# Zehong-Ma/MagCache

Hardware: NVIDIA H100
Metric: denoising_steps_per_sec (higher is better)
Workload: dtype bf16

## Files before the change

### magcache_b200/csrc/gemm_wgmma.cu

```cuda
#include <cstdlib>

#include "common.cuh"
#include "ptx.cuh"
#include "tma_host.cuh"

namespace mc {

TmapCacheEntry* tmap_cache() {
  static TmapCacheEntry table[kTmapCacheSize] = {};
  return table;
}
std::mutex& tmap_cache_mutex() {
  static std::mutex m;
  return m;
}

constexpr int kCluster = 2;
constexpr int kBM = 128, kBK = 64, kStages = 4;
constexpr int kClusterBM = kCluster * kBM;
constexpr int kTileABytes = kBM * kBK * 2;
constexpr int kStagePad = 33;
constexpr int kEpiWarps = 8;
constexpr int kPatchRows = 16;
constexpr int kStagingBytes = kEpiWarps * kPatchRows * kStagePad * 4;
constexpr int kGemmThreads = 128 + 32 * kEpiWarps;
constexpr int kProducerRegs = 40, kConsumerRegs = 232;
template <int BN>
struct GemmTile {
  static constexpr int kTileBBytes = BN * kBK * 2;
  static constexpr int kHalfBBytes = kTileBBytes / kCluster;
  static constexpr int kStageBytes = kTileABytes + kTileBBytes;
  static constexpr int kOffStaging = kStages * kStageBytes;
  static constexpr int kOffBars = kOffStaging + kStagingBytes;
  static constexpr int kSmem = kOffBars + 128;
};

struct GemmParams {
  int M, N, K;
  const float* bias;
  void* out;
  int64_t ldo;
  const float* gate;
  int total_tiles;
};

template <int EPI, int ROWS>
__device__ __forceinline__ void epilogue_patch(const GemmParams& p, const float* stage, int row0, int col0, int lane) {
  const int rows = min(ROWS, p.M - row0);
  if (rows <= 0) return;
  const int col = col0 + lane;
  const bool col_ok = col < p.N;

  if (EPI == MC_EPI_BIAS_GATE_RESID) {
    const float b = (p.bias && col_ok) ? p.bias[col] : 0.f;
    const float g = (p.gate && col_ok) ? p.gate[col] : 1.f;
    float* xcol = static_cast<float*>(p.out) + static_cast<int64_t>(row0) * p.ldo + col;
#pragma unroll
    for (int h = 0; h < ROWS; h += 16) {
      float xv[16];
#pragma unroll
      for (int r = 0; r < 16; ++r) xv[r] = (col_ok && h + r < rows) ? xcol[static_cast<int64_t>(h + r) * p.ldo] : 0.f;
#pragma unroll
      for (int r = 0; r < 16; ++r) {
        const float y = round_bf16(stage[(h + r) * kStagePad + lane] + b);
        xv[r] = __fadd_rn(xv[r], __fmul_rn(y, g));
      }
#pragma unroll
      for (int r = 0; r < 16; ++r)
        if (col_ok && h + r < rows) xcol[static_cast<int64_t>(h + r) * p.ldo] = xv[r];
    }
    return;
  }

  if (EPI == MC_EPI_BIAS_F32) {
    const float b = (p.bias && col_ok) ? p.bias[col] : 0.f;
    float* ocol = static_cast<float*>(p.out) + static_cast<int64_t>(row0) * p.ldo + col;
#pragma unroll
    for (int r = 0; r < ROWS; ++r)
      if (col_ok && r < rows) ocol[static_cast<int64_t>(r) * p.ldo] = stage[r * kStagePad + lane] + b;
    return;
  }

  const int half = lane >> 4, cp = (lane & 15) * 2;
  const int c0 = col0 + cp;
  float b0 = 0.f, b1 = 0.f;
  if (EPI != MC_EPI_ROWBIAS_BF16 && p.bias) {
    if (c0 < p.N) b0 = p.bias[c0];
    if (c0 + 1 < p.N) b1 = p.bias[c0 + 1];
  }
  float g0 = 1.f, g1 = 1.f;
  if (EPI == MC_EPI_BIAS_GATE_RESID_BF16 && p.gate) {
    if (c0 < p.N) g0 = p.gate[c0];
    if (c0 + 1 < p.N) g1 = p.gate[c0 + 1];
  }
  __nv_bfloat16* obase = static_cast<__nv_bfloat16*>(p.out) + static_cast<int64_t>(row0 + half) * p.ldo + c0;
  const float* sbase = stage + half * kStagePad + cp;
  const float* rbias = (EPI == MC_EPI_ROWBIAS_BF16 && p.bias) ? p.bias + row0 + half : nullptr;

  if (rows == ROWS && col0 + 32 <= p.N && (p.ldo & 1) == 0) {
    uint32_t w[ROWS / 2];
#pragma unroll
    for (int i = 0; i < ROWS / 2; ++i) {
      float v0 = sbase[2 * i * kStagePad], v1 = sbase[2 * i * kStagePad + 1];
      if (EPI == MC_EPI_ROWBIAS_BF16) {
        const float rb = rbias ? rbias[2 * i] : 0.f;
        v0 += rb;
        v1 += rb;
      } else {
        v0 += b0;
        v1 += b1;
      }
      if (EPI == MC_EPI_BIAS_GELU_BF16) {
        v0 = gelu_tanh(round_bf16(v0));
        v1 = gelu_tanh(round_bf16(v1));
      }
      if (EPI == MC_EPI_BIAS_GELU_ERF_BF16) {
        v0 = gelu_erf(round_bf16(v0));
        v1 = gelu_erf(round_bf16(v1));
      }
      if (EPI == MC_EPI_BIAS_SILU_BF16) {
        v0 = silu_f(round_bf16(v0));
        v1 = silu_f(round_bf16(v1));
      }
      if (EPI == MC_EPI_BIAS_GATE_RESID_BF16) {
        const uint32_t old = *reinterpret_cast<const uint32_t*>(obase + static_cast<int64_t>(2 * i) * p.ldo);
        v0 = bf16_lo(old) + round_bf16(g0 * round_bf16(v0));
        v1 = bf16_hi(old) + round_bf16(g1 * round_bf16(v1));
      }
      w[i] = pack_bf16x2(v0, v1);
    }
#pragma unroll
    for (int i = 0; i < ROWS / 2; ++i) *reinterpret_cast<uint32_t*>(obase + static_cast<int64_t>(2 * i) * p.ldo) = w[i];
    return;
  }

  const bool pair_ok = (c0 + 1 < p.N) && ((p.ldo & 1) == 0);
  for (int i = 0; i < ROWS / 2; ++i) {
    const int r = 2 * i + half;
    if (r >= rows) continue;
    float v0 = sbase[2 * i * kStagePad], v1 = sbase[2 * i * kStagePad + 1];
    if (EPI == MC_EPI_ROWBIAS_BF16) {
      const float rb = rbias ? rbias[2 * i] : 0.f;
      v0 += rb;
      v1 += rb;
    } else {
      v0 += b0;
      v1 += b1;
    }
    if (EPI == MC_EPI_BIAS_GELU_BF16) {
      v0 = gelu_tanh(round_bf16(v0));
      v1 = gelu_tanh(round_bf16(v1));
    }
    if (EPI == MC_EPI_BIAS_GELU_ERF_BF16) {
      v0 = gelu_erf(round_bf16(v0));
      v1 = gelu_erf(round_bf16(v1));
    }
    if (EPI == MC_EPI_BIAS_SILU_BF16) {
      v0 = silu_f(round_bf16(v0));
      v1 = silu_f(round_bf16(v1));
    }
    __nv_bfloat16* o = obase + static_cast<int64_t>(2 * i) * p.ldo;
    if (EPI == MC_EPI_BIAS_GATE_RESID_BF16) {
      if (c0 < p.N) v0 = __bfloat162float(o[0]) + round_bf16(g0 * round_bf16(v0));
      if (c0 + 1 < p.N) v1 = __bfloat162float(o[1]) + round_bf16(g1 * round_bf16(v1));
    }
    if (pair_ok) {
      *reinterpret_cast<uint32_t*>(o) = pack_bf16x2(v0, v1);
    } else {
      if (c0 < p.N) o[0] = __float2bfloat16_rn(v0);
      if (c0 + 1 < p.N) o[1] = __float2bfloat16_rn(v1);
    }
  }
}

template <int EPI, int kBN>
__global__ void __cluster_dims__(kCluster, 1, 1) __launch_bounds__(kGemmThreads, 1)
    gemm_bf16_kernel(const __grid_constant__ CUtensorMap tmap_a, const __grid_constant__ CUtensorMap tmap_b, const GemmParams p) {
  using T = GemmTile<kBN>;
  constexpr int kStageBytes = T::kStageBytes, kOffStaging = T::kOffStaging, kOffBars = T::kOffBars;
  extern __shared__ __align__(1024) uint8_t smem[];
  float* staging = reinterpret_cast<float*>(smem + kOffStaging);
  uint64_t* full_bar = reinterpret_cast<uint64_t*>(smem + kOffBars);
  uint64_t* empty_bar = full_bar + kStages;

  const int warp = threadIdx.x >> 5, lane = threadIdx.x & 31;
  const int n_tiles = (p.N + kBN - 1) / kBN;
  const int num_kb = (p.K + kBK - 1) / kBK;
  const uint32_t rank = ptx::cluster_ctarank();
  const int cluster = static_cast<int>(ptx::cluster_id_x()), n_clusters = static_cast<int>(ptx::num_clusters_x());
  const int steps = (p.total_tiles - cluster + n_clusters - 1) / n_clusters;

  if (threadIdx.x == 0) {
    if ((ptx::smem_u32(smem) & 1023u) != 0) {
      MC_DIAG("gemm_bf16_kernel: dynamic smem base not 1024-aligned\n");
      __trap();
    }
    ptx::prefetch_tmap(&tmap_a);
    ptx::prefetch_tmap(&tmap_b);
    for (int s = 0; s < kStages; ++s) {
      ptx::mbar_init(&full_bar[s], 1);
      ptx::mbar_init(&empty_bar[s], kCluster * kEpiWarps);
    }
    ptx::fence_mbar_init();
  }
  ptx::cluster_arrive();
  ptx::cluster_wait();

  if (warp < 4) {
    ptx::setmaxnreg_dec<kProducerRegs>();
    if (warp == 0) {
      uint32_t it = 0;
      for (int i = 0; i < steps; ++i) {
        const int tile = cluster + i * n_clusters;
        const int m0 = (tile / n_tiles) * kClusterBM + static_cast<int>(rank) * kBM, n0 = (tile % n_tiles) * kBN;
        const int nb = n0 + static_cast<int>(rank) * (kBN / kCluster);
        for (int kb = 0; kb < num_kb; ++kb, ++it) {
          const int s = it % kStages;
          const uint32_t ph = (it / kStages) & 1;
          ptx::mbar_wait(&empty_bar[s], ph ^ 1);
          if (ptx::elect_one()) {
            uint8_t* sa = smem + s * kStageBytes;
            ptx::mbar_expect_tx(&full_bar[s], kStageBytes);
            ptx::tma_load_2d(sa, &tmap_a, &full_bar[s], kb * kBK, m0);
            ptx::tma_load_2d_multicast(sa + kTileABytes + rank * T::kHalfBBytes, &tmap_b, &full_bar[s], kb * kBK, nb,
                                       static_cast<uint16_t>((1u << kCluster) - 1));
          }
          __syncwarp();
        }
      }
    }
  } else {
    ptx::setmaxnreg_inc<kConsumerRegs>();
    const int wg = (warp >> 2) - 1;
    const int wq = warp & 3;
    float acc[kBN / 2];
    bool timed_out = false;
    for (int i = 0; i < steps; ++i) {
      const int tile = cluster + i * n_clusters;
      const int m0 = (tile / n_tiles) * kClusterBM + static_cast<int>(rank) * kBM, n0 = (tile % n_tiles) * kBN;
      uint32_t it = static_cast<uint32_t>(i) * num_kb;
      int prev_s = -1;
      for (int kb = 0; kb < num_kb; ++kb, ++it) {
        const int s = it % kStages;
        const uint32_t ph = (it / kStages) & 1;
        ptx::mbar_wait_or_flag(&full_bar[s], ph, timed_out);
        const uint32_t sa = ptx::smem_u32(smem + s * kStageBytes);
        const uint64_t da = ptx::gmma_desc_sw128_kmajor(sa + wg * (64 * 128));
        const uint64_t db = ptx::gmma_desc_sw128_kmajor(sa + kTileABytes);
        ptx::wgmma_fence();
#pragma unroll
        for (int k = 0; k < kBK / 16; ++k) {
          if constexpr (kBN == 256) {
            ptx::wgmma_m64n256k16_ss(acc, da + 2 * k, db + 2 * k, (kb | k) != 0 ? 1u : 0u);
          } else {
            ptx::wgmma_m64n128k16_ss(acc, da + 2 * k, db + 2 * k, (kb | k) != 0 ? 1u : 0u);
          }
        }
        ptx::wgmma_commit();
        ptx::wgmma_wait<1>();
        ptx::fence_regs(acc);
        if (prev_s >= 0 && lane == 0)
          for (uint32_t c = 0; c < kCluster; ++c) ptx::mbar_arrive_cluster(&empty_bar[prev_s], c);
        prev_s = s;
      }
      ptx::wgmma_wait<0>();
      ptx::fence_regs(acc);
      if (lane == 0)
        for (uint32_t c = 0; c < kCluster; ++c) ptx::mbar_arrive_cluster(&empty_bar[prev_s], c);

      float* patch = staging + (4 * wg + wq) * kPatchRows * kStagePad;
      const int row0 = m0 + wg * 64 + wq * kPatchRows;
      const int r_lo = lane >> 2;
#pragma unroll
      for (int c = 0; c < kBN / 32; ++c) {
        __syncwarp();
#pragma unroll
        for (int q = 0; q < 4; ++q) {
          const int i = 4 * c + q;
          const int col = 8 * q + 2 * (lane & 3);
          patch[r_lo * kStagePad + col] = acc[4 * i + 0];
          patch[r_lo * kStagePad + col + 1] = acc[4 * i + 1];
          patch[(r_lo + 8) * kStagePad + col] = acc[4 * i + 2];
          patch[(r_lo + 8) * kStagePad + col + 1] = acc[4 * i + 3];
        }
        __syncwarp();
        epilogue_patch<EPI, kPatchRows>(p, patch, row0, n0 + c * 32, lane);
      }
    }
    if (timed_out) __trap();
  }
  ptx::cluster_arrive();
  ptx::cluster_wait();
}

template <int EPI, int BN>
static int32_t max_active_clusters(int* out) {
  static int cached[kMaxDevices] = {};
  const int d = current_device();
  if (cached[d] > 0) {
    *out = cached[d];
    return MC_OK;
  }
  cudaLaunchConfig_t cfg = {};
  cfg.gridDim = dim3(kCluster * num_sms(), 1, 1);
  cfg.blockDim = dim3(kGemmThreads, 1, 1);
  cfg.dynamicSmemBytes = GemmTile<BN>::kSmem;
  int n = 0;
  const cudaError_t e = cudaOccupancyMaxActiveClusters(&n, gemm_bf16_kernel<EPI, BN>, &cfg);
  if (e != cudaSuccess) return cuda_fail(e, "cudaOccupancyMaxActiveClusters(gemm)");
  if (n < 1) {
    set_error("gemm_bf16_kernel: no cluster of %d CTAs with %d B of shared memory fits on this device", kCluster, GemmTile<BN>::kSmem);
    return MC_ERR_CUDA;
  }
  cached[d] = n;
  *out = n;
  return MC_OK;
}

template <int EPI, int BN>
static int32_t launch_gemm_bn(const CUtensorMap& ta, const CUtensorMap& tb, GemmParams p, cudaStream_t s) {
  static PerDeviceOnce once;
  int32_t rc = set_max_smem_once(gemm_bf16_kernel<EPI, BN>, GemmTile<BN>::kSmem, once, "cudaFuncSetAttribute(gemm smem)");
  if (rc) return rc;
  int clusters = 0;
  rc = max_active_clusters<EPI, BN>(&clusters);
  if (rc) return rc;
  const int m_tiles = (p.M + kClusterBM - 1) / kClusterBM, n_tiles = (p.N + BN - 1) / BN;
  const int total = m_tiles * n_tiles;
  p.total_tiles = total;
  const int grid = kCluster * (total < clusters ? total : clusters);
  gemm_bf16_kernel<EPI, BN><<<grid, kGemmThreads, GemmTile<BN>::kSmem, s>>>(ta, tb, p);
  MC_CHECK_LAUNCH("gemm_bf16_kernel launch");
  return MC_OK;
}

static int pick_bn(int M, int N) {
  const char* e = getenv("MC_GEMM_BN");
  if (e && *e) {
    const int v = atoi(e);
    if (v == 128 || v == 256) return v;
  }
  const int64_t sms = num_sms(), m_tiles = (M + 127) / 128;
  const int64_t t256 = m_tiles * ((N + 255) / 256), t128 = m_tiles * ((N + 127) / 128);
  const int64_t cost256 = ((t256 + sms - 1) / sms) * 100, cost128 = ((t128 + sms - 1) / sms) * 62;
  return cost128 * 100 <= cost256 * 92 ? 128 : 256;
}

}

extern "C" int32_t mc_gemm_bf16(const void* A, int64_t lda, const void* B, int64_t ldb, int32_t M, int32_t N, int32_t K,
                                const float* bias, int32_t epilogue, void* out, int64_t ldo, const float* gate, void* stream) {
  MC_CHECK_ARG(A && B && out, "mc_gemm_bf16: null pointer");
  MC_CHECK_ARG(M >= 1 && N >= 1 && K >= 8, "mc_gemm_bf16: M=%d N=%d K=%d", M, N, K);
  MC_CHECK_ARG(K % 8 == 0 && lda % 8 == 0 && ldb % 8 == 0 && lda >= K && ldb >= K, "mc_gemm_bf16: K/lda/ldb must be multiples of 8 (16-byte TMA pitch)");
  MC_CHECK_ARG(mc::aligned16(A) && mc::aligned16(B) && mc::aligned16(out), "mc_gemm_bf16: A/B/out must be 16-byte aligned");
  MC_CHECK_ARG(ldo >= N, "mc_gemm_bf16: ldo=%lld < N=%d", static_cast<long long>(ldo), N);
  CUtensorMap ta, tb;
  int32_t rc = mc::make_tmap_bf16_2d(&ta, A, static_cast<uint64_t>(M), static_cast<uint64_t>(K), static_cast<uint64_t>(lda), mc::kBM, mc::kBK);
  if (rc) return rc;
  const int bn = mc::pick_bn(M, N);
  rc = mc::make_tmap_bf16_2d(&tb, B, static_cast<uint64_t>(N), static_cast<uint64_t>(K), static_cast<uint64_t>(ldb), bn / mc::kCluster,
                             mc::kBK);
  if (rc) return rc;
  mc::GemmParams p{M, N, K, bias, out, ldo, gate, 0};
  cudaStream_t s = static_cast<cudaStream_t>(stream);
#define MC_GEMM_CASE(E) \
  case E: return bn == 128 ? mc::launch_gemm_bn<E, 128>(ta, tb, p, s) : mc::launch_gemm_bn<E, 256>(ta, tb, p, s)
  switch (epilogue) {
    MC_GEMM_CASE(MC_EPI_BIAS_BF16);
    MC_GEMM_CASE(MC_EPI_BIAS_GELU_BF16);
    MC_GEMM_CASE(MC_EPI_BIAS_GATE_RESID);
    MC_GEMM_CASE(MC_EPI_ROWBIAS_BF16);
    MC_GEMM_CASE(MC_EPI_BIAS_F32);
    MC_GEMM_CASE(MC_EPI_BIAS_GELU_ERF_BF16);
    MC_GEMM_CASE(MC_EPI_BIAS_GATE_RESID_BF16);
    MC_GEMM_CASE(MC_EPI_BIAS_SILU_BF16);
#undef MC_GEMM_CASE
    default:
      mc::set_error("mc_gemm_bf16: unknown epilogue %d", epilogue);
      return MC_ERR_INVALID;
  }
}
```

### magcache_b200/csrc/ptx.cuh

```cuda
#pragma once
#include <cstdint>
#include <cuda_runtime.h>

namespace ptx {

__device__ __forceinline__ uint32_t smem_u32(const void* p) {
  return static_cast<uint32_t>(__cvta_generic_to_shared(p));
}

__device__ __forceinline__ void mbar_init(uint64_t* bar, uint32_t count) {
  asm volatile("mbarrier.init.shared::cta.b64 [%0], %1;" ::"r"(smem_u32(bar)), "r"(count) : "memory");
}
__device__ __forceinline__ void fence_mbar_init() {
  asm volatile("fence.mbarrier_init.release.cluster;" ::: "memory");
}
__device__ __forceinline__ void mbar_expect_tx(uint64_t* bar, uint32_t bytes) {
  asm volatile("mbarrier.arrive.expect_tx.shared::cta.b64 _, [%0], %1;" ::"r"(smem_u32(bar)), "r"(bytes) : "memory");
}
__device__ __forceinline__ void mbar_arrive(uint64_t* bar) {
  asm volatile("mbarrier.arrive.shared::cta.b64 _, [%0];" ::"r"(smem_u32(bar)) : "memory");
}
__device__ __forceinline__ bool mbar_try_wait(uint64_t* bar, uint32_t parity) {
  uint32_t ok;
  asm volatile(
      "{\n"
      ".reg .pred p;\n"
      "mbarrier.try_wait.parity.shared::cta.b64 p, [%1], %2;\n"
      "selp.u32 %0, 1, 0, p;\n"
      "}\n"
      : "=r"(ok)
      : "r"(smem_u32(bar)), "r"(parity)
      : "memory");
  return ok != 0;
}
#ifndef MC_DEVICE_DIAG
#define MC_DEVICE_DIAG 0
#endif
#if MC_DEVICE_DIAG
#define MC_DIAG(...) printf(__VA_ARGS__)
#else
#define MC_DIAG(...) ((void)0)
#endif

#ifndef MC_MBAR_TIMEOUT_CYCLES
#define MC_MBAR_TIMEOUT_CYCLES (4000000000ll)
#endif
__device__ __forceinline__ void mbar_wait(uint64_t* bar, uint32_t parity) {
  if (mbar_try_wait(bar, parity)) return;
  const long long t0 = clock64();
  while (!mbar_try_wait(bar, parity)) {
    if (clock64() - t0 > MC_MBAR_TIMEOUT_CYCLES) {
      MC_DIAG("mbar_wait timeout: block (%d,%d,%d) thread %d bar smem+%u parity %u\n", blockIdx.x, blockIdx.y, blockIdx.z,
              threadIdx.x, smem_u32(bar), parity);
      __trap();
    }
  }
}
__device__ __forceinline__ void mbar_wait_or_flag(uint64_t* bar, uint32_t parity, bool& timed_out) {
  if (timed_out || mbar_try_wait(bar, parity)) return;
  const long long t0 = clock64();
  while (!mbar_try_wait(bar, parity)) {
    if (clock64() - t0 > MC_MBAR_TIMEOUT_CYCLES) {
      MC_DIAG("mbar_wait timeout: block (%d,%d,%d) thread %d bar smem+%u parity %u\n", blockIdx.x, blockIdx.y, blockIdx.z,
              threadIdx.x, smem_u32(bar), parity);
      timed_out = true;
      return;
    }
  }
}

__device__ __forceinline__ void named_bar_sync(uint32_t id, uint32_t count) {
  asm volatile("bar.sync %0, %1;" ::"r"(id), "r"(count) : "memory");
}
__device__ __forceinline__ void named_bar_arrive(uint32_t id, uint32_t count) {
  asm volatile("bar.arrive %0, %1;" ::"r"(id), "r"(count) : "memory");
}

__device__ __forceinline__ uint32_t cluster_ctarank() {
  uint32_t r;
  asm volatile("mov.u32 %0, %%cluster_ctarank;" : "=r"(r));
  return r;
}
__device__ __forceinline__ uint32_t cluster_id_x() {
  uint32_t r;
  asm volatile("mov.u32 %0, %%clusterid.x;" : "=r"(r));
  return r;
}
__device__ __forceinline__ uint32_t num_clusters_x() {
  uint32_t r;
  asm volatile("mov.u32 %0, %%nclusterid.x;" : "=r"(r));
  return r;
}
__device__ __forceinline__ void mbar_arrive_cluster(uint64_t* bar, uint32_t cta) {
  asm volatile(
      "{\n"
      ".reg .b32 ra;\n"
      "mapa.shared::cluster.u32 ra, %0, %1;\n"
      "mbarrier.arrive.shared::cluster.b64 _, [ra];\n"
      "}\n"
      ::"r"(smem_u32(bar)), "r"(cta)
      : "memory");
}
__device__ __forceinline__ void cluster_arrive() { asm volatile("barrier.cluster.arrive.release.aligned;" ::: "memory"); }
__device__ __forceinline__ void cluster_wait() { asm volatile("barrier.cluster.wait.acquire.aligned;" ::: "memory"); }

__device__ __forceinline__ bool elect_one() {
  uint32_t pred;
  asm volatile(
      "{\n"
      ".reg .pred P;\n"
      "elect.sync _|P, 0xffffffff;\n"
      "selp.u32 %0, 1, 0, P;\n"
      "}\n"
      : "=r"(pred));
  return pred != 0;
}

__device__ __forceinline__ void fence_proxy_async_smem() {
  asm volatile("fence.proxy.async.shared::cta;" ::: "memory");
}

__device__ __forceinline__ void prefetch_tmap(const void* tmap) {
  asm volatile("prefetch.tensormap [%0];" ::"l"(reinterpret_cast<uint64_t>(tmap)) : "memory");
}
__device__ __forceinline__ void tma_load_2d(void* smem_dst, const void* tmap, uint64_t* bar, int32_t c0, int32_t c1) {
  asm volatile(
      "cp.async.bulk.tensor.2d.shared::cluster.global.mbarrier::complete_tx::bytes [%0], [%1, {%3, %4}], [%2];"
      ::"r"(smem_u32(smem_dst)), "l"(reinterpret_cast<uint64_t>(tmap)), "r"(smem_u32(bar)), "r"(c0), "r"(c1)
      : "memory");
}

__device__ __forceinline__ void tma_load_2d_multicast(void* smem_dst, const void* tmap, uint64_t* bar, int32_t c0, int32_t c1,
                                                      uint16_t cta_mask) {
  asm volatile(
      "cp.async.bulk.tensor.2d.shared::cluster.global.mbarrier::complete_tx::bytes.multicast::cluster [%0], [%1, {%3, %4}], [%2], %5;"
      ::"r"(smem_u32(smem_dst)), "l"(reinterpret_cast<uint64_t>(tmap)), "r"(smem_u32(bar)), "r"(c0), "r"(c1), "h"(cta_mask)
      : "memory");
}

__device__ __forceinline__ void bulk_load_1d(void* smem_dst, const void* gmem_src, uint32_t bytes, uint64_t* bar) {
  asm volatile("cp.async.bulk.shared::cluster.global.mbarrier::complete_tx::bytes [%0], [%1], %2, [%3];" ::"r"(smem_u32(smem_dst)),
               "l"(reinterpret_cast<uint64_t>(gmem_src)), "r"(bytes), "r"(smem_u32(bar))
               : "memory");
}

__device__ __forceinline__ uint64_t gmma_desc_sw128_kmajor(uint32_t smem_addr) {
  uint64_t d = 0;
  d |= static_cast<uint64_t>((smem_addr & 0x3FFFFu) >> 4);
  d |= static_cast<uint64_t>(1) << 16;
  d |= static_cast<uint64_t>(1024 >> 4) << 32;
  d |= static_cast<uint64_t>(1) << 62;
  return d;
}
__device__ __forceinline__ uint64_t gmma_desc_sw128_mnmajor(uint32_t smem_addr, uint32_t lbo_bytes, uint32_t sbo_bytes = 1024) {
  uint64_t d = 0;
  d |= static_cast<uint64_t>((smem_addr & 0x3FFFFu) >> 4);
  d |= static_cast<uint64_t>((lbo_bytes >> 4) & 0x3FFFu) << 16;
  d |= static_cast<uint64_t>((sbo_bytes >> 4) & 0x3FFFu) << 32;
  d |= static_cast<uint64_t>(1) << 62;
  return d;
}
__device__ __forceinline__ void wgmma_fence() { asm volatile("wgmma.fence.sync.aligned;" ::: "memory"); }
__device__ __forceinline__ void wgmma_commit() { asm volatile("wgmma.commit_group.sync.aligned;" ::: "memory"); }
template <int N>
__device__ __forceinline__ void wgmma_wait() {
  asm volatile("wgmma.wait_group.sync.aligned %0;" ::"n"(N) : "memory");
}
template <int N>
__device__ __forceinline__ void fence_regs(float (&d)[N]) {
#pragma unroll
  for (int i = 0; i < N; ++i) asm volatile("" : "+f"(d[i])::"memory");
}

__device__ __forceinline__ void wgmma_m64n64k16_ss(float (&d)[32], uint64_t adesc, uint64_t bdesc, uint32_t accumulate) {
  asm volatile(
      "{\n"
      ".reg .pred p;\n"
      "setp.ne.b32 p, %34, 0;\n"
      "wgmma.mma_async.sync.aligned.m64n64k16.f32.bf16.bf16 "
      "{%0, %1, %2, %3, %4, %5, %6, %7, %8, %9, %10, %11, %12, %13, %14, %15, %16, %17, %18, %19, %20, %21, %22, %23, %24, %25, %26, %27, %28, %29, %30, %31}, "
      "%32, %33, p, 1, 1, 0, 0;\n"
      "}\n"
      : "+f"(d[0]), "+f"(d[1]), "+f"(d[2]), "+f"(d[3]), "+f"(d[4]), "+f"(d[5]), "+f"(d[6]), "+f"(d[7]), "+f"(d[8]), "+f"(d[9]), "+f"(d[10]), "+f"(d[11]), "+f"(d[12]), "+f"(d[13]), "+f"(d[14]), "+f"(d[15]), "+f"(d[16]), "+f"(d[17]), "+f"(d[18]), "+f"(d[19]), "+f"(d[20]), "+f"(d[21]), "+f"(d[22]), "+f"(d[23]), "+f"(d[24]), "+f"(d[25]), "+f"(d[26]), "+f"(d[27]), "+f"(d[28]), "+f"(d[29]), "+f"(d[30]), "+f"(d[31])
      : "l"(adesc), "l"(bdesc), "r"(accumulate));
}
__device__ __forceinline__ void wgmma_m64n128k16_ss(float (&d)[64], uint64_t adesc, uint64_t bdesc, uint32_t accumulate) {
  asm volatile(
      "{\n"
      ".reg .pred p;\n"
      "setp.ne.b32 p, %66, 0;\n"
      "wgmma.mma_async.sync.aligned.m64n128k16.f32.bf16.bf16 "
      "{%0, %1, %2, %3, %4, %5, %6, %7, %8, %9, %10, %11, %12, %13, %14, %15, %16, %17, %18, %19, %20, %21, %22, %23, %24, %25, %26, %27, %28, %29, %30, %31, %32, %33, %34, %35, %36, %37, %38, %39, %40, %41, %42, %43, %44, %45, %46, %47, %48, %49, %50, %51, %52, %53, %54, %55, %56, %57, %58, %59, %60, %61, %62, %63}, "
      "%64, %65, p, 1, 1, 0, 0;\n"
      "}\n"
      : "+f"(d[0]), "+f"(d[1]), "+f"(d[2]), "+f"(d[3]), "+f"(d[4]), "+f"(d[5]), "+f"(d[6]), "+f"(d[7]), "+f"(d[8]), "+f"(d[9]), "+f"(d[10]), "+f"(d[11]), "+f"(d[12]), "+f"(d[13]), "+f"(d[14]), "+f"(d[15]), "+f"(d[16]), "+f"(d[17]), "+f"(d[18]), "+f"(d[19]), "+f"(d[20]), "+f"(d[21]), "+f"(d[22]), "+f"(d[23]), "+f"(d[24]), "+f"(d[25]), "+f"(d[26]), "+f"(d[27]), "+f"(d[28]), "+f"(d[29]), "+f"(d[30]), "+f"(d[31]), "+f"(d[32]), "+f"(d[33]), "+f"(d[34]), "+f"(d[35]), "+f"(d[36]), "+f"(d[37]), "+f"(d[38]), "+f"(d[39]), "+f"(d[40]), "+f"(d[41]), "+f"(d[42]), "+f"(d[43]), "+f"(d[44]), "+f"(d[45]), "+f"(d[46]), "+f"(d[47]), "+f"(d[48]), "+f"(d[49]), "+f"(d[50]), "+f"(d[51]), "+f"(d[52]), "+f"(d[53]), "+f"(d[54]), "+f"(d[55]), "+f"(d[56]), "+f"(d[57]), "+f"(d[58]), "+f"(d[59]), "+f"(d[60]), "+f"(d[61]), "+f"(d[62]), "+f"(d[63])
      : "l"(adesc), "l"(bdesc), "r"(accumulate));
}
__device__ __forceinline__ void wgmma_m64n256k16_ss(float (&d)[128], uint64_t adesc, uint64_t bdesc, uint32_t accumulate) {
  asm volatile(
      "{\n"
      ".reg .pred p;\n"
      "setp.ne.b32 p, %130, 0;\n"
      "wgmma.mma_async.sync.aligned.m64n256k16.f32.bf16.bf16 "
      "{%0, %1, %2, %3, %4, %5, %6, %7, %8, %9, %10, %11, %12, %13, %14, %15, %16, %17, %18, %19, %20, %21, %22, %23, %24, %25, %26, %27, %28, %29, %30, %31, %32, %33, %34, %35, %36, %37, %38, %39, %40, %41, %42, %43, %44, %45, %46, %47, %48, %49, %50, %51, %52, %53, %54, %55, %56, %57, %58, %59, %60, %61, %62, %63, %64, %65, %66, %67, %68, %69, %70, %71, %72, %73, %74, %75, %76, %77, %78, %79, %80, %81, %82, %83, %84, %85, %86, %87, %88, %89, %90, %91, %92, %93, %94, %95, %96, %97, %98, %99, %100, %101, %102, %103, %104, %105, %106, %107, %108, %109, %110, %111, %112, %113, %114, %115, %116, %117, %118, %119, %120, %121, %122, %123, %124, %125, %126, %127}, "
      "%128, %129, p, 1, 1, 0, 0;\n"
      "}\n"
      : "+f"(d[0]), "+f"(d[1]), "+f"(d[2]), "+f"(d[3]), "+f"(d[4]), "+f"(d[5]), "+f"(d[6]), "+f"(d[7]), "+f"(d[8]), "+f"(d[9]), "+f"(d[10]), "+f"(d[11]), "+f"(d[12]), "+f"(d[13]), "+f"(d[14]), "+f"(d[15]), "+f"(d[16]), "+f"(d[17]), "+f"(d[18]), "+f"(d[19]), "+f"(d[20]), "+f"(d[21]), "+f"(d[22]), "+f"(d[23]), "+f"(d[24]), "+f"(d[25]), "+f"(d[26]), "+f"(d[27]), "+f"(d[28]), "+f"(d[29]), "+f"(d[30]), "+f"(d[31]), "+f"(d[32]), "+f"(d[33]), "+f"(d[34]), "+f"(d[35]), "+f"(d[36]), "+f"(d[37]), "+f"(d[38]), "+f"(d[39]), "+f"(d[40]), "+f"(d[41]), "+f"(d[42]), "+f"(d[43]), "+f"(d[44]), "+f"(d[45]), "+f"(d[46]), "+f"(d[47]), "+f"(d[48]), "+f"(d[49]), "+f"(d[50]), "+f"(d[51]), "+f"(d[52]), "+f"(d[53]), "+f"(d[54]), "+f"(d[55]), "+f"(d[56]), "+f"(d[57]), "+f"(d[58]), "+f"(d[59]), "+f"(d[60]), "+f"(d[61]), "+f"(d[62]), "+f"(d[63]), "+f"(d[64]), "+f"(d[65]), "+f"(d[66]), "+f"(d[67]), "+f"(d[68]), "+f"(d[69]), "+f"(d[70]), "+f"(d[71]), "+f"(d[72]), "+f"(d[73]), "+f"(d[74]), "+f"(d[75]), "+f"(d[76]), "+f"(d[77]), "+f"(d[78]), "+f"(d[79]), "+f"(d[80]), "+f"(d[81]), "+f"(d[82]), "+f"(d[83]), "+f"(d[84]), "+f"(d[85]), "+f"(d[86]), "+f"(d[87]), "+f"(d[88]), "+f"(d[89]), "+f"(d[90]), "+f"(d[91]), "+f"(d[92]), "+f"(d[93]), "+f"(d[94]), "+f"(d[95]), "+f"(d[96]), "+f"(d[97]), "+f"(d[98]), "+f"(d[99]), "+f"(d[100]), "+f"(d[101]), "+f"(d[102]), "+f"(d[103]), "+f"(d[104]), "+f"(d[105]), "+f"(d[106]), "+f"(d[107]), "+f"(d[108]), "+f"(d[109]), "+f"(d[110]), "+f"(d[111]), "+f"(d[112]), "+f"(d[113]), "+f"(d[114]), "+f"(d[115]), "+f"(d[116]), "+f"(d[117]), "+f"(d[118]), "+f"(d[119]), "+f"(d[120]), "+f"(d[121]), "+f"(d[122]), "+f"(d[123]), "+f"(d[124]), "+f"(d[125]), "+f"(d[126]), "+f"(d[127])
      : "l"(adesc), "l"(bdesc), "r"(accumulate));
}
__device__ __forceinline__ void wgmma_m64n128k16_rs_tb(float (&d)[64], const uint32_t (&a)[4], uint64_t bdesc, uint32_t accumulate) {
  asm volatile(
      "{\n"
      ".reg .pred p;\n"
      "setp.ne.b32 p, %69, 0;\n"
      "wgmma.mma_async.sync.aligned.m64n128k16.f32.bf16.bf16 "
      "{%0, %1, %2, %3, %4, %5, %6, %7, %8, %9, %10, %11, %12, %13, %14, %15, %16, %17, %18, %19, %20, %21, %22, %23, %24, %25, %26, %27, %28, %29, %30, %31, %32, %33, %34, %35, %36, %37, %38, %39, %40, %41, %42, %43, %44, %45, %46, %47, %48, %49, %50, %51, %52, %53, %54, %55, %56, %57, %58, %59, %60, %61, %62, %63}, "
      "{%64, %65, %66, %67}, %68, p, 1, 1, 1;\n"
      "}\n"
      : "+f"(d[0]), "+f"(d[1]), "+f"(d[2]), "+f"(d[3]), "+f"(d[4]), "+f"(d[5]), "+f"(d[6]), "+f"(d[7]), "+f"(d[8]), "+f"(d[9]), "+f"(d[10]), "+f"(d[11]), "+f"(d[12]), "+f"(d[13]), "+f"(d[14]), "+f"(d[15]), "+f"(d[16]), "+f"(d[17]), "+f"(d[18]), "+f"(d[19]), "+f"(d[20]), "+f"(d[21]), "+f"(d[22]), "+f"(d[23]), "+f"(d[24]), "+f"(d[25]), "+f"(d[26]), "+f"(d[27]), "+f"(d[28]), "+f"(d[29]), "+f"(d[30]), "+f"(d[31]), "+f"(d[32]), "+f"(d[33]), "+f"(d[34]), "+f"(d[35]), "+f"(d[36]), "+f"(d[37]), "+f"(d[38]), "+f"(d[39]), "+f"(d[40]), "+f"(d[41]), "+f"(d[42]), "+f"(d[43]), "+f"(d[44]), "+f"(d[45]), "+f"(d[46]), "+f"(d[47]), "+f"(d[48]), "+f"(d[49]), "+f"(d[50]), "+f"(d[51]), "+f"(d[52]), "+f"(d[53]), "+f"(d[54]), "+f"(d[55]), "+f"(d[56]), "+f"(d[57]), "+f"(d[58]), "+f"(d[59]), "+f"(d[60]), "+f"(d[61]), "+f"(d[62]), "+f"(d[63])
      : "r"(a[0]), "r"(a[1]), "r"(a[2]), "r"(a[3]), "l"(bdesc), "r"(accumulate));
}


template <int N>
__device__ __forceinline__ void setmaxnreg_inc() {
  asm volatile("setmaxnreg.inc.sync.aligned.u32 %0;" ::"n"(N));
}
template <int N>
__device__ __forceinline__ void setmaxnreg_dec() {
  asm volatile("setmaxnreg.dec.sync.aligned.u32 %0;" ::"n"(N));
}

__device__ __forceinline__ float ex2_approx(float x) {
  float y;
  asm("ex2.approx.ftz.f32 %0, %1;" : "=f"(y) : "f"(x));
  return y;
}
__device__ __forceinline__ float ex2_emul(float x) {
  const float kMagic = 12582912.0f;
  x = fmaxf(x, -126.0f);
  const float t = __fadd_rd(x, kMagic);
  const float f = x - __fadd_rn(t, -kMagic);
  float p = __fmaf_rn(0.077119089663028717041015625f, f, 0.227564394474029541015625f);
  p = __fmaf_rn(p, f, 0.695146143436431884765625f);
  p = __fmaf_rn(p, f, 1.0f);
  return __int_as_float(__float_as_int(p) + (__float_as_int(t) << 23));
}
__device__ __forceinline__ uint4 ld_nc_v4(const void* p) {
  uint4 r;
  asm volatile("ld.global.nc.L1::no_allocate.v4.u32 {%0, %1, %2, %3}, [%4];" : "=r"(r.x), "=r"(r.y), "=r"(r.z), "=r"(r.w) : "l"(p));
  return r;
}
__device__ __forceinline__ void st_na_v4(void* p, const uint4& v) {
  asm volatile("st.global.L1::no_allocate.v4.u32 [%0], {%1, %2, %3, %4};" ::"l"(p), "r"(v.x), "r"(v.y), "r"(v.z), "r"(v.w) : "memory");
}

__device__ __forceinline__ void ld_nc_v8_f32(const float* p, float (&f)[8]) {
  asm volatile("ld.global.nc.L1::no_allocate.v4.f32 {%0, %1, %2, %3}, [%4];" : "=f"(f[0]), "=f"(f[1]), "=f"(f[2]), "=f"(f[3]) : "l"(p));
  asm volatile("ld.global.nc.L1::no_allocate.v4.f32 {%0, %1, %2, %3}, [%4];" : "=f"(f[4]), "=f"(f[5]), "=f"(f[6]), "=f"(f[7]) : "l"(p + 4));
}
__device__ __forceinline__ void ld_v8_f32(const float* p, float (&f)[8]) {
  asm volatile("ld.global.v4.f32 {%0, %1, %2, %3}, [%4];" : "=f"(f[0]), "=f"(f[1]), "=f"(f[2]), "=f"(f[3]) : "l"(p) : "memory");
  asm volatile("ld.global.v4.f32 {%0, %1, %2, %3}, [%4];" : "=f"(f[4]), "=f"(f[5]), "=f"(f[6]), "=f"(f[7]) : "l"(p + 4) : "memory");
}
__device__ __forceinline__ void st_na_v8_f32(float* p, const float (&f)[8]) {
  asm volatile("st.global.L1::no_allocate.v4.f32 [%0], {%1, %2, %3, %4};" ::"l"(p), "f"(f[0]), "f"(f[1]), "f"(f[2]), "f"(f[3]) : "memory");
  asm volatile("st.global.L1::no_allocate.v4.f32 [%0], {%1, %2, %3, %4};" ::"l"(p + 4), "f"(f[4]), "f"(f[5]), "f"(f[6]), "f"(f[7]) : "memory");
}
}
```

### magcache_b200/csrc/tma_host.cuh

```cuda
#pragma once
#include <cuda.h>
#include <mutex>
#include <cuda_runtime.h>

#include "common.cuh"

namespace mc {

typedef CUresult (*PFN_encodeTiled)(CUtensorMap*, CUtensorMapDataType, cuuint32_t, void*, const cuuint64_t*, const cuuint64_t*,
                                    const cuuint32_t*, const cuuint32_t*, CUtensorMapInterleave, CUtensorMapSwizzle,
                                    CUtensorMapL2promotion, CUtensorMapFloatOOBfill);

inline PFN_encodeTiled get_encode_tiled() {
  static PFN_encodeTiled fn = nullptr;
  if (fn == nullptr) {
    void* p = nullptr;
    cudaDriverEntryPointQueryResult qres;
    cudaError_t e = cudaGetDriverEntryPoint("cuTensorMapEncodeTiled", &p, cudaEnableDefault, &qres);
    if (e != cudaSuccess || qres != cudaDriverEntryPointSuccess || p == nullptr) {
      set_error("cudaGetDriverEntryPoint(cuTensorMapEncodeTiled) failed: %s", cudaGetErrorString(e));
      return nullptr;
    }
    fn = reinterpret_cast<PFN_encodeTiled>(p);
  }
  return fn;
}

struct TmapKey {
  const void* base;
  uint64_t rows, cols, ld;
  uint32_t box_rows, box_cols;
  bool operator==(const TmapKey& o) const {
    return base == o.base && rows == o.rows && cols == o.cols && ld == o.ld && box_rows == o.box_rows && box_cols == o.box_cols;
  }
};
struct TmapCacheEntry {
  TmapKey key;
  CUtensorMap map;
  bool valid;
};
constexpr int kTmapCacheSize = 1024;
TmapCacheEntry* tmap_cache();
std::mutex& tmap_cache_mutex();

inline int32_t make_tmap_bf16_2d_uncached(CUtensorMap* map, const void* base, uint64_t rows, uint64_t cols, uint64_t ld, uint32_t box_rows,
                                          uint32_t box_cols);

inline int32_t make_tmap_bf16_2d(CUtensorMap* map, const void* base, uint64_t rows, uint64_t cols, uint64_t ld, uint32_t box_rows,
                                 uint32_t box_cols) {
  const TmapKey key{base, rows, cols, ld, box_rows, box_cols};
  uint64_t h = reinterpret_cast<uint64_t>(base) >> 4;
  h ^= rows * 0x9E3779B97F4A7C15ull;
  h ^= (cols << 20) ^ (ld << 40) ^ (static_cast<uint64_t>(box_rows) << 8) ^ box_cols;
  h ^= h >> 29;
  h *= 0xBF58476D1CE4E5B9ull;
  h ^= h >> 32;
  TmapCacheEntry& e = tmap_cache()[h % kTmapCacheSize];
  {
    std::lock_guard<std::mutex> g(tmap_cache_mutex());
    if (e.valid && e.key == key) {
      *map = e.map;
      return MC_OK;
    }
  }
  const int32_t rc = make_tmap_bf16_2d_uncached(map, base, rows, cols, ld, box_rows, box_cols);
  if (rc == MC_OK) {
    std::lock_guard<std::mutex> g(tmap_cache_mutex());
    e.key = key;
    e.map = *map;
    e.valid = true;
  }
  return rc;
}

inline int32_t make_tmap_bf16_2d_uncached(CUtensorMap* map, const void* base, uint64_t rows, uint64_t cols, uint64_t ld, uint32_t box_rows,
                                          uint32_t box_cols) {
  PFN_encodeTiled enc = get_encode_tiled();
  if (!enc) return MC_ERR_CUDA;
  cuuint64_t gdim[2] = {cols, rows};
  cuuint64_t gstride[1] = {ld * 2};
  cuuint32_t box[2] = {box_cols, box_rows};
  cuuint32_t estr[2] = {1, 1};
  CUresult r = enc(map, CU_TENSOR_MAP_DATA_TYPE_BFLOAT16, 2, const_cast<void*>(base), gdim, gstride, box, estr,
                   CU_TENSOR_MAP_INTERLEAVE_NONE, CU_TENSOR_MAP_SWIZZLE_128B, CU_TENSOR_MAP_L2_PROMOTION_L2_256B,
                   CU_TENSOR_MAP_FLOAT_OOB_FILL_NONE);
  if (r != CUDA_SUCCESS) {
    set_error("cuTensorMapEncodeTiled failed (CUresult %d): base=%p rows=%llu cols=%llu ld=%llu box=[%u,%u]", static_cast<int>(r), base,
              static_cast<unsigned long long>(rows), static_cast<unsigned long long>(cols), static_cast<unsigned long long>(ld), box_rows,
              box_cols);
    return MC_ERR_CUDA;
  }
  return MC_OK;
}

}
```

Measured before the change: 1.283.

## Write GEMM epilogue through swizzled smem slabs with TMA stores and reduce-adds

Adds a TMA-based epilogue: each consumer warpgroup applies bias, gate and activation in registers, writes 64x128-byte swizzled slabs to double-buffered shared memory, and issues bulk tensor stores. The gate-residual fp32 case uses a TMA reduce-add instead of read-modify-write. This replaces the per-warp padded staging and scalar global stores, cutting store instruction count and letting the epilogue overlap stores with the next slab. It adds named-barrier syncs per slab and an output tensor map built per call, and falls back to the old path for unaligned outputs or the bf16 residual epilogue.

Measured after the change: 1.318 (median of 6 runs). +2.8%, better.

```diff
diff --git a/magcache_b200/csrc/gemm_wgmma.cu b/magcache_b200/csrc/gemm_wgmma.cu
--- a/magcache_b200/csrc/gemm_wgmma.cu
+++ b/magcache_b200/csrc/gemm_wgmma.cu
@@ -23,6 +23,10 @@
 constexpr int kEpiWarps = 8;
 constexpr int kPatchRows = 16;
 constexpr int kStagingBytes = kEpiWarps * kPatchRows * kStagePad * 4;
+constexpr int kSlabBytes = 64 * 128;
+constexpr int kSlabsBytes = 2 * 2 * kSlabBytes;
+static_assert(kStagingBytes <= kSlabsBytes, "patches");
+constexpr int kEpiBarrier0 = 1;
 constexpr int kGemmThreads = 128 + 32 * kEpiWarps;
 constexpr int kProducerRegs = 40, kConsumerRegs = 232;
 template <int BN>
@@ -30,8 +34,8 @@
   static constexpr int kTileBBytes = BN * kBK * 2;
   static constexpr int kHalfBBytes = kTileBBytes / kCluster;
   static constexpr int kStageBytes = kTileABytes + kTileBBytes;
-  static constexpr int kOffStaging = kStages * kStageBytes;
-  static constexpr int kOffBars = kOffStaging + kStagingBytes;
+  static constexpr int kOffSlabs = kStages * kStageBytes;
+  static constexpr int kOffBars = kOffSlabs + kSlabsBytes;
   static constexpr int kSmem = kOffBars + 128;
 };
 
@@ -174,12 +178,97 @@
 }
 
 template <int EPI, int kBN>
+__device__ __forceinline__ void epilogue_tma(const GemmParams& p, const CUtensorMap* tmap_out, const float (&acc)[kBN / 2], uint8_t* slabs,
+                                             int row0, int n0, int wg, int wq, int lane) {
+  constexpr bool kF32 = EPI == MC_EPI_BIAS_GATE_RESID || EPI == MC_EPI_BIAS_F32;
+  constexpr int kEsz = kF32 ? 4 : 2, kSlabCols = 128 / kEsz;
+  static_assert((kBN / kSlabCols) % 2 == 0, "slab c of every tile must use buffer c & 1");
+  const bool leader = wq == 0 && lane == 0;
+  const int r0 = wq * 16 + (lane >> 2);
+  const int cl = 2 * (lane & 3);
+  float rb0 = 0.f, rb1 = 0.f;
+  if (EPI == MC_EPI_ROWBIAS_BF16 && p.bias) {
+    if (row0 + r0 < p.M) rb0 = p.bias[row0 + r0];
+    if (row0 + r0 + 8 < p.M) rb1 = p.bias[row0 + r0 + 8];
+  }
+  constexpr int kQ = kSlabCols / 8;
+  float bv[2][2 * kQ], gv[2][2 * kQ];
+  auto load_cols = [&](int c, float(&b)[2 * kQ], float(&g)[2 * kQ]) {
+#pragma unroll
+    for (int e = 0; e < 2 * kQ; ++e) {
+      const int col = n0 + c * kSlabCols + 8 * (e >> 1) + cl + (e & 1);
+      b[e] = (EPI != MC_EPI_ROWBIAS_BF16 && p.bias && col < p.N) ? p.bias[col] : 0.f;
+      g[e] = (EPI == MC_EPI_BIAS_GATE_RESID && p.gate && col < p.N) ? p.gate[col] : 1.f;
+    }
+  };
+  load_cols(0, bv[0], gv[0]);
+#pragma unroll
+  for (int c = 0; c < kBN / kSlabCols; ++c) {
+    if (c + 1 < kBN / kSlabCols) load_cols(c + 1, bv[(c + 1) & 1], gv[(c + 1) & 1]);
+    const float(&bc)[2 * kQ] = bv[c & 1];
+    const float(&gc)[2 * kQ] = gv[c & 1];
+    uint8_t* slab = slabs + (c & 1) * kSlabBytes;
+    if (leader) ptx::bulk_wait_group_read<1>();
+    ptx::named_bar_sync(kEpiBarrier0 + wg, 128);
+#pragma unroll
+    for (int q = 0; q < kQ; ++q) {
+      const int i = c * kQ + q;
+      float v[4] = {acc[4 * i], acc[4 * i + 1], acc[4 * i + 2], acc[4 * i + 3]};
+      if (EPI == MC_EPI_ROWBIAS_BF16) {
+        v[0] += rb0;
+        v[1] += rb0;
+        v[2] += rb1;
+        v[3] += rb1;
+      } else {
+        v[0] += bc[2 * q];
+        v[1] += bc[2 * q + 1];
+        v[2] += bc[2 * q];
+        v[3] += bc[2 * q + 1];
+      }
+      if (EPI == MC_EPI_BIAS_GATE_RESID) {
+        v[0] = __fmul_rn(round_bf16(v[0]), gc[2 * q]);
+        v[1] = __fmul_rn(round_bf16(v[1]), gc[2 * q + 1]);
+        v[2] = __fmul_rn(round_bf16(v[2]), gc[2 * q]);
+        v[3] = __fmul_rn(round_bf16(v[3]), gc[2 * q + 1]);
+      }
+#pragma unroll
+      for (int j = 0; j < 4; ++j) {
+        if (EPI == MC_EPI_BIAS_GELU_BF16) v[j] = gelu_tanh(round_bf16(v[j]));
+        if (EPI == MC_EPI_BIAS_GELU_ERF_BF16) v[j] = gelu_erf(round_bf16(v[j]));
+        if (EPI == MC_EPI_BIAS_SILU_BF16) v[j] = silu_f(round_bf16(v[j]));
+      }
+      const int byte = (8 * q + cl) * kEsz;
+      const int chunk = ((byte >> 4) ^ (lane >> 2)) << 4;
+#pragma unroll
+      for (int h = 0; h < 2; ++h) {
+        uint8_t* dst = slab + (r0 + 8 * h) * 128 + chunk + (byte & 15);
+        if constexpr (kF32) {
+          *reinterpret_cast<float2*>(dst) = make_float2(v[2 * h], v[2 * h + 1]);
+        } else {
+          *reinterpret_cast<uint32_t*>(dst) = pack_bf16x2(v[2 * h], v[2 * h + 1]);
+        }
+      }
+    }
+    ptx::fence_proxy_async_smem();
+    ptx::named_bar_sync(kEpiBarrier0 + wg, 128);
+    if (leader) {
+      if constexpr (EPI == MC_EPI_BIAS_GATE_RESID) {
+        ptx::tma_reduce_add_2d(tmap_out, slab, n0 + c * kSlabCols, row0);
+      } else {
+        ptx::tma_store_2d(tmap_out, slab, n0 + c * kSlabCols, row0);
+      }
+      ptx::bulk_commit_group();
+    }
+  }
+}
+
+template <int EPI, int kBN, bool kTmaOut>
 __global__ void __cluster_dims__(kCluster, 1, 1) __launch_bounds__(kGemmThreads, 1)
-    gemm_bf16_kernel(const __grid_constant__ CUtensorMap tmap_a, const __grid_constant__ CUtensorMap tmap_b, const GemmParams p) {
+    gemm_bf16_kernel(const __grid_constant__ CUtensorMap tmap_a, const __grid_constant__ CUtensorMap tmap_b,
+                     const __grid_constant__ CUtensorMap tmap_out, const GemmParams p) {
   using T = GemmTile<kBN>;
-  constexpr int kStageBytes = T::kStageBytes, kOffStaging = T::kOffStaging, kOffBars = T::kOffBars;
+  constexpr int kStageBytes = T::kStageBytes, kOffSlabs = T::kOffSlabs, kOffBars = T::kOffBars;
   extern __shared__ __align__(1024) uint8_t smem[];
-  float* staging = reinterpret_cast<float*>(smem + kOffStaging);
   uint64_t* full_bar = reinterpret_cast<uint64_t*>(smem + kOffBars);
   uint64_t* empty_bar = full_bar + kStages;
 
@@ -197,6 +286,7 @@
     }
     ptx::prefetch_tmap(&tmap_a);
     ptx::prefetch_tmap(&tmap_b);
+    if (kTmaOut) ptx::prefetch_tmap(&tmap_out);
     for (int s = 0; s < kStages; ++s) {
       ptx::mbar_init(&full_bar[s], 1);
       ptx::mbar_init(&empty_bar[s], kCluster * kEpiWarps);
@@ -268,7 +358,11 @@
       if (lane == 0)
         for (uint32_t c = 0; c < kCluster; ++c) ptx::mbar_arrive_cluster(&empty_bar[prev_s], c);
 
-      float* patch = staging + (4 * wg + wq) * kPatchRows * kStagePad;
+      if constexpr (kTmaOut) {
+        epilogue_tma<EPI, kBN>(p, &tmap_out, acc, smem + kOffSlabs + wg * 2 * kSlabBytes, m0 + wg * 64, n0, wg, wq, lane);
+        continue;
+      }
+      float* patch = reinterpret_cast<float*>(smem + kOffSlabs) + (4 * wg + wq) * kPatchRows * kStagePad;
       const int row0 = m0 + wg * 64 + wq * kPatchRows;
       const int r_lo = lane >> 2;
 #pragma unroll
@@ -287,13 +381,14 @@
         epilogue_patch<EPI, kPatchRows>(p, patch, row0, n0 + c * 32, lane);
       }
     }
+    if (kTmaOut && wq == 0 && lane == 0) ptx::bulk_wait_group<0>();
     if (timed_out) __trap();
   }
   ptx::cluster_arrive();
   ptx::cluster_wait();
 }
 
-template <int EPI, int BN>
+template <int EPI, int BN, bool TMA>
 static int32_t max_active_clusters(int* out) {
   static int cached[kMaxDevices] = {};
   const int d = current_device();
@@ -306,7 +401,7 @@
   cfg.blockDim = dim3(kGemmThreads, 1, 1);
   cfg.dynamicSmemBytes = GemmTile<BN>::kSmem;
   int n = 0;
-  const cudaError_t e = cudaOccupancyMaxActiveClusters(&n, gemm_bf16_kernel<EPI, BN>, &cfg);
+  const cudaError_t e = cudaOccupancyMaxActiveClusters(&n, gemm_bf16_kernel<EPI, BN, TMA>, &cfg);
   if (e != cudaSuccess) return cuda_fail(e, "cudaOccupancyMaxActiveClusters(gemm)");
   if (n < 1) {
     set_error("gemm_bf16_kernel: no cluster of %d CTAs with %d B of shared memory fits on this device", kCluster, GemmTile<BN>::kSmem);
@@ -317,21 +412,30 @@
   return MC_OK;
 }
 
-template <int EPI, int BN>
-static int32_t launch_gemm_bn(const CUtensorMap& ta, const CUtensorMap& tb, GemmParams p, cudaStream_t s) {
+template <int EPI, int BN, bool TMA>
+static int32_t launch_gemm_bn(const CUtensorMap& ta, const CUtensorMap& tb, const CUtensorMap& to, GemmParams p, cudaStream_t s) {
   static PerDeviceOnce once;
-  int32_t rc = set_max_smem_once(gemm_bf16_kernel<EPI, BN>, GemmTile<BN>::kSmem, once, "cudaFuncSetAttribute(gemm smem)");
+  int32_t rc = set_max_smem_once(gemm_bf16_kernel<EPI, BN, TMA>, GemmTile<BN>::kSmem, once, "cudaFuncSetAttribute(gemm smem)");
   if (rc) return rc;
   int clusters = 0;
-  rc = max_active_clusters<EPI, BN>(&clusters);
+  rc = max_active_clusters<EPI, BN, TMA>(&clusters);
   if (rc) return rc;
   const int m_tiles = (p.M + kClusterBM - 1) / kClusterBM, n_tiles = (p.N + BN - 1) / BN;
   const int total = m_tiles * n_tiles;
   p.total_tiles = total;
   const int grid = kCluster * (total < clusters ? total : clusters);
-  gemm_bf16_kernel<EPI, BN><<<grid, kGemmThreads, GemmTile<BN>::kSmem, s>>>(ta, tb, p);
+  gemm_bf16_kernel<EPI, BN, TMA><<<grid, kGemmThreads, GemmTile<BN>::kSmem, s>>>(ta, tb, to, p);
   MC_CHECK_LAUNCH("gemm_bf16_kernel launch");
   return MC_OK;
+}
+
+template <int EPI>
+static int32_t launch_gemm(const CUtensorMap& ta, const CUtensorMap& tb, const CUtensorMap& to, const GemmParams& p, int bn, bool tma_out,
+                           cudaStream_t s) {
+  if constexpr (EPI != MC_EPI_BIAS_GATE_RESID_BF16) {
+    if (tma_out) return bn == 128 ? launch_gemm_bn<EPI, 128, true>(ta, tb, to, p, s) : launch_gemm_bn<EPI, 256, true>(ta, tb, to, p, s);
+  }
+  return bn == 128 ? launch_gemm_bn<EPI, 128, false>(ta, tb, to, p, s) : launch_gemm_bn<EPI, 256, false>(ta, tb, to, p, s);
 }
 
 static int pick_bn(int M, int N) {
@@ -362,10 +466,18 @@
   rc = mc::make_tmap_bf16_2d(&tb, B, static_cast<uint64_t>(N), static_cast<uint64_t>(K), static_cast<uint64_t>(ldb), bn / mc::kCluster,
                              mc::kBK);
   if (rc) return rc;
+  const bool f32_out = epilogue == MC_EPI_BIAS_GATE_RESID || epilogue == MC_EPI_BIAS_F32;
+  const uint32_t esize = f32_out ? 4 : 2;
+  const bool tma_out = epilogue != MC_EPI_BIAS_GATE_RESID_BF16 && (ldo * esize) % 16 == 0 && (N * esize) % 16 == 0;
+  CUtensorMap to = {};
+  if (tma_out) {
+    rc = mc::make_tmap_2d(&to, out, esize, static_cast<uint64_t>(M), static_cast<uint64_t>(N), static_cast<uint64_t>(ldo), 64, 128 / esize);
+    if (rc) return rc;
+  }
   mc::GemmParams p{M, N, K, bias, out, ldo, gate, 0};
   cudaStream_t s = static_cast<cudaStream_t>(stream);
 #define MC_GEMM_CASE(E) \
-  case E: return bn == 128 ? mc::launch_gemm_bn<E, 128>(ta, tb, p, s) : mc::launch_gemm_bn<E, 256>(ta, tb, p, s)
+  case E: return mc::launch_gemm<E>(ta, tb, to, p, bn, tma_out, s)
   switch (epilogue) {
     MC_GEMM_CASE(MC_EPI_BIAS_BF16);
     MC_GEMM_CASE(MC_EPI_BIAS_GELU_BF16);
diff --git a/magcache_b200/csrc/ptx.cuh b/magcache_b200/csrc/ptx.cuh
--- a/magcache_b200/csrc/ptx.cuh
+++ b/magcache_b200/csrc/ptx.cuh
@@ -144,6 +144,26 @@
                : "memory");
 }
 
+__device__ __forceinline__ void tma_store_2d(const void* tmap, const void* smem_src, int32_t c0, int32_t c1) {
+  asm volatile("cp.async.bulk.tensor.2d.global.shared::cta.bulk_group [%0, {%2, %3}], [%1];"
+               ::"l"(reinterpret_cast<uint64_t>(tmap)), "r"(smem_u32(smem_src)), "r"(c0), "r"(c1)
+               : "memory");
+}
+__device__ __forceinline__ void tma_reduce_add_2d(const void* tmap, const void* smem_src, int32_t c0, int32_t c1) {
+  asm volatile("cp.reduce.async.bulk.tensor.2d.global.shared::cta.add.tile.bulk_group [%0, {%2, %3}], [%1];"
+               ::"l"(reinterpret_cast<uint64_t>(tmap)), "r"(smem_u32(smem_src)), "r"(c0), "r"(c1)
+               : "memory");
+}
+__device__ __forceinline__ void bulk_commit_group() { asm volatile("cp.async.bulk.commit_group;" ::: "memory"); }
+template <int N>
+__device__ __forceinline__ void bulk_wait_group_read() {
+  asm volatile("cp.async.bulk.wait_group.read %0;" ::"n"(N) : "memory");
+}
+template <int N>
+__device__ __forceinline__ void bulk_wait_group() {
+  asm volatile("cp.async.bulk.wait_group %0;" ::"n"(N) : "memory");
+}
+
 __device__ __forceinline__ uint64_t gmma_desc_sw128_kmajor(uint32_t smem_addr) {
   uint64_t d = 0;
   d |= static_cast<uint64_t>((smem_addr & 0x3FFFFu) >> 4);
diff --git a/magcache_b200/csrc/tma_host.cuh b/magcache_b200/csrc/tma_host.cuh
--- a/magcache_b200/csrc/tma_host.cuh
+++ b/magcache_b200/csrc/tma_host.cuh
@@ -29,9 +29,10 @@
 struct TmapKey {
   const void* base;
   uint64_t rows, cols, ld;
-  uint32_t box_rows, box_cols;
+  uint32_t box_rows, box_cols, esize;
   bool operator==(const TmapKey& o) const {
-    return base == o.base && rows == o.rows && cols == o.cols && ld == o.ld && box_rows == o.box_rows && box_cols == o.box_cols;
+    return base == o.base && rows == o.rows && cols == o.cols && ld == o.ld && box_rows == o.box_rows && box_cols == o.box_cols &&
+           esize == o.esize;
   }
 };
 struct TmapCacheEntry {
@@ -43,15 +44,15 @@
 TmapCacheEntry* tmap_cache();
 std::mutex& tmap_cache_mutex();
 
-inline int32_t make_tmap_bf16_2d_uncached(CUtensorMap* map, const void* base, uint64_t rows, uint64_t cols, uint64_t ld, uint32_t box_rows,
-                                          uint32_t box_cols);
+inline int32_t make_tmap_2d_uncached(CUtensorMap* map, const void* base, uint32_t esize, uint64_t rows, uint64_t cols, uint64_t ld,
+                                     uint32_t box_rows, uint32_t box_cols);
 
-inline int32_t make_tmap_bf16_2d(CUtensorMap* map, const void* base, uint64_t rows, uint64_t cols, uint64_t ld, uint32_t box_rows,
-                                 uint32_t box_cols) {
-  const TmapKey key{base, rows, cols, ld, box_rows, box_cols};
+inline int32_t make_tmap_2d(CUtensorMap* map, const void* base, uint32_t esize, uint64_t rows, uint64_t cols, uint64_t ld,
+                            uint32_t box_rows, uint32_t box_cols) {
+  const TmapKey key{base, rows, cols, ld, box_rows, box_cols, esize};
   uint64_t h = reinterpret_cast<uint64_t>(base) >> 4;
   h ^= rows * 0x9E3779B97F4A7C15ull;
-  h ^= (cols << 20) ^ (ld << 40) ^ (static_cast<uint64_t>(box_rows) << 8) ^ box_cols;
+  h ^= (cols << 20) ^ (ld << 40) ^ (static_cast<uint64_t>(box_rows) << 8) ^ box_cols ^ (static_cast<uint64_t>(esize) << 60);
   h ^= h >> 29;
   h *= 0xBF58476D1CE4E5B9ull;
   h ^= h >> 32;
@@ -63,7 +64,7 @@
       return MC_OK;
     }
   }
-  const int32_t rc = make_tmap_bf16_2d_uncached(map, base, rows, cols, ld, box_rows, box_cols);
+  const int32_t rc = make_tmap_2d_uncached(map, base, esize, rows, cols, ld, box_rows, box_cols);
   if (rc == MC_OK) {
     std::lock_guard<std::mutex> g(tmap_cache_mutex());
     e.key = key;
@@ -73,21 +74,26 @@
   return rc;
 }
 
-inline int32_t make_tmap_bf16_2d_uncached(CUtensorMap* map, const void* base, uint64_t rows, uint64_t cols, uint64_t ld, uint32_t box_rows,
-                                          uint32_t box_cols) {
+inline int32_t make_tmap_bf16_2d(CUtensorMap* map, const void* base, uint64_t rows, uint64_t cols, uint64_t ld, uint32_t box_rows,
+                                 uint32_t box_cols) {
+  return make_tmap_2d(map, base, 2, rows, cols, ld, box_rows, box_cols);
+}
+
+inline int32_t make_tmap_2d_uncached(CUtensorMap* map, const void* base, uint32_t esize, uint64_t rows, uint64_t cols, uint64_t ld,
+                                     uint32_t box_rows, uint32_t box_cols) {
   PFN_encodeTiled enc = get_encode_tiled();
   if (!enc) return MC_ERR_CUDA;
   cuuint64_t gdim[2] = {cols, rows};
-  cuuint64_t gstride[1] = {ld * 2};
+  cuuint64_t gstride[1] = {ld * esize};
   cuuint32_t box[2] = {box_cols, box_rows};
   cuuint32_t estr[2] = {1, 1};
-  CUresult r = enc(map, CU_TENSOR_MAP_DATA_TYPE_BFLOAT16, 2, const_cast<void*>(base), gdim, gstride, box, estr,
-                   CU_TENSOR_MAP_INTERLEAVE_NONE, CU_TENSOR_MAP_SWIZZLE_128B, CU_TENSOR_MAP_L2_PROMOTION_L2_256B,
-                   CU_TENSOR_MAP_FLOAT_OOB_FILL_NONE);
+  const CUtensorMapDataType dt = esize == 4 ? CU_TENSOR_MAP_DATA_TYPE_FLOAT32 : CU_TENSOR_MAP_DATA_TYPE_BFLOAT16;
+  CUresult r = enc(map, dt, 2, const_cast<void*>(base), gdim, gstride, box, estr, CU_TENSOR_MAP_INTERLEAVE_NONE,
+                   CU_TENSOR_MAP_SWIZZLE_128B, CU_TENSOR_MAP_L2_PROMOTION_L2_256B, CU_TENSOR_MAP_FLOAT_OOB_FILL_NONE);
   if (r != CUDA_SUCCESS) {
-    set_error("cuTensorMapEncodeTiled failed (CUresult %d): base=%p rows=%llu cols=%llu ld=%llu box=[%u,%u]", static_cast<int>(r), base,
-              static_cast<unsigned long long>(rows), static_cast<unsigned long long>(cols), static_cast<unsigned long long>(ld), box_rows,
-              box_cols);
+    set_error("cuTensorMapEncodeTiled failed (CUresult %d): base=%p esize=%u rows=%llu cols=%llu ld=%llu box=[%u,%u]", static_cast<int>(r),
+              base, esize, static_cast<unsigned long long>(rows), static_cast<unsigned long long>(cols), static_cast<unsigned long long>(ld),
+              box_rows, box_cols);
     return MC_ERR_CUDA;
   }
   return MC_OK;
```
